# nvpro-samples/vk_gaussian_splatting

Measured on AMD Instinct MI355X. Metric: frames/s @1920x1080 + sorted Gsplats/s, garden-sized scene, higher is better.
Workload: dtype f32; 1 GPU; syn_garden N=5830000 x 1 instance(s) SH deg 3, storage sh/rgba format 0/0, 1920x1080, 64-pose orbit r=4 h=1.5 fov60, GPU radix sort, cull at dist (configs[2]); partition=single GPU

## Files before the change

vk_gaussian_splatting_amd/csrc/api_frame.hip:

```cpp
#include <cmath>

#include "scene_state.h"

int mgs_frame_set_occluder(MgsScene s, const float* depthDevice, const float* colorDevice, int width, int height)
{
  if(!s)
  {
    setError("mgs_frame_set_occluder: null handle");
    return MGS_ERR_INVALID_ARG;
  }
  if(!depthDevice)
  {
    s->occ.depth = s->occ.color = nullptr;
    s->occ.w = s->occ.h = 0;
    return MGS_OK;
  }
  if(width <= 0 || height <= 0)
  {
    setError("mgs_frame_set_occluder: width and height must be positive");
    return MGS_ERR_INVALID_ARG;
  }
  s->occ.depth = depthDevice;
  s->occ.color = colorDevice;
  s->occ.w     = width;
// ... 319 lines not shown
    if((rc = fb.pairVal0.ensure(cap))) return rc;
    if((rc = fb.pairKey1.ensure(cap))) return rc;
    if((rc = fb.chunkStart.ensure(cap / kPart + 4))) return rc;
    if((rc = fb.splatOffset.ensure(s->d->totalSplats))) return rc;
  }
  return ensureFrameImage(s, fp.p, F, std::max<uint32_t>(fp.nTiles, 256u), fp.occ.depth);
}

ProjectLaunch projectLaunch(MgsScene s, const FrameArgs& A, bool full, bool gpuSort)
{
  FrameBuffers& fb = s->fb;
  ProjectLaunch L{};
  L.dArgs           = fb.dArgs.p;
  L.totalPartitions = A.f.totalPartitions;
  L.full            = full;
  L.ctr             = fb.ctr.p;
  L.slotPairs       = fb.pairB.p;
  L.slotCount       = fb.slotCount.p;
  L.rec             = fb.rec.p;
  L.recGut          = fb.recGut.p;
  L.rect            = fb.rect.p;
  L.slotHist2       = fb.slotHist2.p;
  L.top16Rec        = fb.top16Rec.p;
  L.top16Count      = gpuSort ? fb.top16Count.p : nullptr;
  L.osPlan          = &fb.plans.p->os;
  L.order           = fb.prjOrder.p;
  return L;
}

static int issueSort(const FramePass& fp, hipStream_t st)
// ... 162 lines not shown
  return MGS_OK;
}

static GraphCache::Key graphKey(const FramePass& fp)
{
  const FrameConst& F = fp.A->f;
  GraphCache::Key   key;
  std::memset(&key, 0, sizeof(key));
  int32_t isoBits;
  std::memcpy(&isoBits, &F.depthIsoThreshold, 4);
  const int32_t kv[16] = {F.width, F.height, F.stripRow0, F.stripRow1, F.binShiftX, F.binShiftY, F.partitionCull, F.alphaMode,
                          F.debugFlags & (2 | 4), F.surfaceOutputs, fp.half, F.nInstances, F.shDegree, isoBits,
                          F.pipeline, F.stochastic | (F.dofMode << 1) | (F.temporalSampling << 2) | ((F.pipeline == 1 && F.kernelDegree != 2) ? 8 : 0) |
                              ((F.pipeline == 1 && F.normalMethod == 1) ? 16 : 0) |
                              (F.lightingMode << 5) |
                              (F.rideShift << 8) | (F.rideShapes << 16) | (F.rideSplit << 24)};
  std::memcpy(key.v, kv, sizeof(kv));
  key.p[0] = fp.s->fb.image.p;
  key.p[1] = fp.s->surf.depth.p;
  key.p[2] = fp.occ.depth;
  key.p[3] = fp.occ.color;
  return key;
}

static int launchFrame(const FramePass& fp, bool timed)
{
  GraphCache& graphs = fp.s->graphs;
  if(tuning().useGraph && graphs.ok && !timed && !fp.cpuMode)
  {
    const GraphCache::Key key  = graphKey(fp);
    hipGraphExec_t        exec = graphs.find(key);
// ... 367 lines not shown
```

vk_gaussian_splatting_amd/csrc/api_frameargs.hip:

```cpp
#include <cmath>

#include "scene_state.h"

void mgs_frame_params_default(MgsFrameParams* p)
{
  if(!p)
    return;
  std::memset(p, 0, sizeof(*p));
  const float id[16] = {1, 0, 0, 0, 0, 1, 0, 0, 0, 0, 1, 0, 0, 0, 0, 1};
  std::memcpy(p->view, id, sizeof(id));
  std::memcpy(p->proj, id, sizeof(id));
  p->width                = 1920;
  p->height               = 1080;
  p->splat_scale          = 1.0f;
  p->frustum_dilation     = 0.2f;
  p->alpha_cull_threshold = 1.0f / 255.0f;
  p->sh_degree            = 3;
  p->sort_mode            = MGS_SORT_GPU_RADIX;
  p->frustum_culling      = MGS_CULL_AT_DIST;
  p->target_format        = MGS_TARGET_RGBA16F;
  p->alpha_mode           = MGS_ALPHA_COVERAGE;
  p->size_culling_min_pixels = 1.0f;
  p->cpu_lazy_sort           = 1;
  p->thin_particle_threshold = 1e-6f;
// ... 126 lines not shown
  F.binsX     = (F.tilesX + (1 << bsx) - 1) >> bsx;
  F.binsY     = (F.tilesY + (1 << bsy) - 1) >> bsy;
  return MGS_OK;
}

static void fillInstanceConst(const MgsFrameParams* p, const Instance& I, const DeviceSet& d, InstanceConst& C)
{
  C.centers = d.centers;
  C.cov6    = d.cov6;
  C.rgba    = d.rgba;
  C.sh      = d.sh;
  C.partBox = d.partBox;
  C.maxScale = d.maxScale;
  C.scales    = d.scales;
  C.alpha     = d.alpha;
  C.rgbaF32   = d.rgbaF32;
  C.rotations = d.rotations;
  {
    auto len3 = [&](int c) { return std::sqrt((I.M[4 * c] * I.M[4 * c] + I.M[4 * c + 1] * I.M[4 * c + 1]) + I.M[4 * c + 2] * I.M[4 * c + 2]); };
    C.modelAxisMax = std::max(len3(0), std::max(len3(1), len3(2)));
  }
  std::memcpy(C.model, I.M, sizeof(C.model));
  mat4Mul(p->view, I.M, C.modelView);
  float inv[16], cam[4] = {p->camera_pos[0], p->camera_pos[1], p->camera_pos[2], 1.0f}, cm[4];
  mat4Inverse(I.M, inv);
  std::memcpy(C.modelInv, inv, sizeof(inv));
  mat4MulVec4(inv, cam, cm);
  C.camModel[0]  = cm[0];
  C.camModel[1]  = cm[1];
  C.camModel[2]  = cm[2];
// ... 139 lines not shown
  F.totalPartitions = s->d->totalParts;
  F.partitionCull   = F.cullMode == MGS_CULL_AT_DIST ? 1 : 0;
  uint32_t offset = 0, block = 0;
  for(int k = 0; k < F.nInstances; ++k)
  {
    const DeviceSet& d = s->d->sets[s->d->instances[k].set];
    InstanceConst&   C = A.inst[k];
    fillInstanceConst(p, s->d->instances[k], d, C);
    C.globalOffset = offset;
    C.blockBegin   = block;
    C.shDegree     = d.shDegree;
    C.shStride     = d.shPitch;
    offset += d.count;
    block += (d.count + kPart - 1) / kPart;
  }
  return MGS_OK;
}
```

vk_gaussian_splatting_amd/csrc/api_scene.hip:

```cpp
#include <cmath>

#include "scene_state.h"

static void materialDefault(MgsMaterial& m)
{
  std::memset(&m, 0, sizeof(m));
  m.emission[0] = m.emission[1] = m.emission[2] = 1.0f;
}
static MaterialDev materialToDevice(const MgsMaterial& m)
{
  MaterialDev d{};
  std::memcpy(d.ambient, m.ambient, 12);
  std::memcpy(d.diffuse, m.diffuse, 12);
  std::memcpy(d.specular, m.specular, 12);
  std::memcpy(d.emission, m.emission, 12);
  d.shininess = m.shininess;
  auto len = [](const float* v) { return std::sqrt(v[0] * v[0] + v[1] * v[1] + v[2] * v[2]); };
  d.needShading = (len(m.diffuse) > 0.001f || len(m.ambient) > 0.001f || len(m.specular) > 0.001f) ? 1 : 0;
  return d;
}

static int mgs_scene_create_impl(int device, MgsScene* out)
{
  if(!out)
  {
    setError("mgs_scene_create: null argument");
    return MGS_ERR_INVALID_ARG;
  }
  int count = 0;
  if(hipGetDeviceCount(&count) != hipSuccess || count == 0)
  {
    setError("mgs_scene_create: no HIP device available — the MI355X path has no CPU fallback");
    return MGS_ERR_DEVICE;
  }
  if(device < 0 || device >= count)
  {
// ... 41 lines not shown
}
int mgs_scene_create(int device, MgsScene* out)
{
  return guarded("mgs_scene_create", [&] { return mgs_scene_create_impl(device, out); });
}

static void freeSet(DeviceSet& d)
{
  if(d.centers) (void)hipFree(d.centers);
  if(d.cov6) (void)hipFree(d.cov6);
  if(d.rgba) (void)hipFree(d.rgba);
  if(d.sh) (void)hipFree(d.sh);
  if(d.partBox) (void)hipFree(d.partBox);
  if(d.maxScale) (void)hipFree(d.maxScale);
  if(d.alpha) (void)hipFree(d.alpha);
  if(d.rgbaF32 && (void*)d.rgbaF32 != d.rgba) (void)hipFree(d.rgbaF32);
  d.rgbaF32 = nullptr;
  if(d.scales) (void)hipFree(d.scales);
  if(d.rotations) (void)hipFree(d.rotations);
  d.centers = d.cov6 = d.partBox = d.maxScale = d.scales = d.rotations = d.alpha = nullptr;
  d.rgba = d.sh = nullptr;
  d.shFormat = d.rgbaFormat = -1;
}

SceneData::~SceneData()
{
  (void)hipSetDevice(device);
  for(auto& d : sets)
    freeSet(d);
  compInst.release();
  lightTab.release();
  for(auto& m : meshes)
    m.release();
  meshTab.release();
  bvh.release();
// ... 75 lines not shown
  {
    setError("mgs_scene_set_list_capacity: null scene");
    return MGS_ERR_INVALID_ARG;
  }
  s->listCapacityOverride = entries;
  s->wsEpoch              = ~0ull;
  return MGS_OK;
}

static uint64_t setBytes(const DeviceSet& d)
{
  if(!d.centers)
    return 0;
  const uint64_t n   = d.count;
  const uint64_t fmt[3] = {4, 2, 1};
  uint64_t       b   = n * (12 + 24 + 4 + 4 + 12 + 16) + ((n + kPart - 1) / kPart) * 32;
  b += n * 4 * fmt[d.rgbaFormat] + (d.rgbaFormat != MGS_FORMAT_FLOAT32 ? n * 16 : 0);
  b += d.sh ? n * (uint64_t)d.shPitch * fmt[d.shFormat] : 0;
  return b;
}
int mgs_scene_memory_usage(MgsScene s, uint64_t* sceneBytes, uint64_t* workingBytes)
{
  if(!s)
  {
    setError("mgs_scene_memory_usage: null scene");
    return MGS_ERR_INVALID_ARG;
  }
  if(sceneBytes)
  {
    uint64_t b = s->d->compInst.bytes() + s->d->lightTab.bytes() + s->d->meshTab.bytes() + s->d->bvh.bytes();
    for(const auto& m : s->d->meshes)
// ... 369 lines not shown
      std::vector<float> al(n);
      if(rgbaFormat != MGS_FORMAT_FLOAT32)
        parallelBatches(n * 4, [&](size_t i) {
          re[i] = rgbaFormat == MGS_FORMAT_FLOAT16 ? halfToFloat(floatToHalf(re[i])) : (float)toUint8(re[i], 0.f, 1.f) / 255.0f;
        });
      parallelBatches(n, [&](size_t i) { al[i] = re[4 * i + 3]; });
      if(rgbaFormat == MGS_FORMAT_FLOAT32)
        d.rgbaF32 = static_cast<float*>(d.rgba);
      else
      {
        HIPCHK(hipMalloc((void**)&d.rgbaF32, n * 4 * sizeof(float)));
        HIPCHK(hipMemcpy(d.rgbaF32, re.data(), n * 4 * sizeof(float), hipMemcpyHostToDevice));
      }
      HIPCHK(hipMalloc((void**)&d.alpha, n * sizeof(float)));
      HIPCHK(hipMemcpy(d.alpha, al.data(), n * sizeof(float), hipMemcpyHostToDevice));
    }
    if(d.shStride)
    {
      std::vector<float> sh, padded;
      buildShInterleaved(h, sh);
      d.shPitch = 48;
      padded.assign(n * (size_t)d.shPitch, 0.f);
      const int stride = d.shStride;
      parallelBatches(n, [&](size_t i) {
        std::memcpy(&padded[i * (size_t)d.shPitch], &sh[(size_t)perm[i] * (size_t)stride], sizeof(float) * stride);
      });
      int rc = uploadFormatted(padded, shFormat, true, &d.sh);
      if(rc != MGS_OK)
        return rc;
    }
// ... 255 lines not shown
```

vk_gaussian_splatting_amd/csrc/device_types.h:

```cpp
#pragma once
#include <cstdint>

namespace mgs {

constexpr int kMaxInstances       = 256;
constexpr int kMaxInlineInstances = 16;
constexpr int kMaxLights          = 64;
constexpr int kTilePx             = 16;

enum : uint32_t {
  kErrPairOverflow  = 1u << 0,
  kErrSpinTimeout   = 1u << 1,
  kErrSortOverflow  = 1u << 2,
};

struct InstanceConst
{
  const float* centers;
  const float* cov6;
  const void*  rgba;
  const float* rgbaF32;
  const float* alpha;
  const float* maxScale;
  const float* partBox;
  const void*  sh;
  const float* scales;
  const float* rotations;
  float        model[16];
  float        modelInv[16];
  float        modelView[16];
  float        camModel[3];
  float        modelAxisMax;
  float        modelScale;
  uint32_t     count;
  uint32_t     modelIsIdentity;
  uint32_t     modelIsAffine;
  uint32_t     globalOffset;
// ... 39 lines not shown
  float    gutFocal[2];
  float    gutMaxAngle;
  float    viewInv[16], projInv[16];
  int32_t  stochastic;
  int32_t  dofMode;
  int32_t  frameSampleId;
  int32_t  temporalSampling;
  float    focusDist, aperture;
  int32_t  kernelDegree;
  int32_t  normalMethod;
  int32_t  rideShift;
  int32_t  rideShapes;
  uint32_t rideEscape;
  int32_t  perspAffine;
  int32_t  rideSplit;
  int32_t  lightingMode;
  float    cameraPos[3];
  float    lightViewInv[16], lightProjInv[16];
};

struct FrameArgs
{
  FrameConst    f;
  InstanceConst inst[kMaxInstances];
};

struct CompositeArgs
{
  int32_t width, height;
  int32_t tilesX;
// ... 222 lines not shown
```

vk_gaussian_splatting_amd/csrc/k_project.hip:

```cpp
#include <cstdio>
#include <cstdlib>
#include <vector>
#include "kernels_common.h"
#include "launchers.h"
#include "slot_emit.h"
#include "partition_cull.h"

namespace mgs {

#ifndef MGS_PRJ_THREADS
#define MGS_PRJ_THREADS 256
#endif
constexpr int kPrjThreads = MGS_PRJ_THREADS;
constexpr int kPrjWaves   = kPrjThreads / 64;
constexpr int kPrjItems   = 2048 / kPrjThreads;
constexpr int kPrjPart    = kPrjThreads * kPrjItems;
static_assert(kPrjItems * kPrjWaves == 32 && kPrjPart == 2048, "the round x wave table of scanRoundWaveCounts has 32 entries");

struct Projected
{
  SplatRec rec;
  uint32_t rect;
};

struct SplatFetch
{
  float  alpha;
  float  px, py, pz;
  float4 cA;
  float2 cB;
};
__device__ __forceinline__ SplatFetch fetchSplat(const InstanceConst& I, uint32_t li)
{
  SplatFetch f;
  f.alpha = I.alpha[li];
  f.px  = I.centers[3 * (size_t)li + 0];
  f.py  = I.centers[3 * (size_t)li + 1];
  f.pz  = I.centers[3 * (size_t)li + 2];
  f.cA  = reinterpret_cast<const float4*>(I.cov6)[li];
  f.cB  = reinterpret_cast<const float2*>(I.cov6 + 4 * (size_t)I.count)[li];
  return f;
}

__device__ __forceinline__ float fastRcp(float x) { return __builtin_amdgcn_rcpf(x); }
__device__ __forceinline__ float fastSqrt(float x) { return __builtin_amdgcn_sqrtf(x); }

__device__ __forceinline__ bool projectSplat(const FrameConst& F, const InstanceConst& I, int instIdx, const SplatFetch& in,
                                             Projected& out)
{
  float4       col = make_float4(0.f, 0.f, 0.f, in.alpha);
  const float  px = in.px, py = in.py, pz = in.pz;
  const float4 cA = in.cA;
  const float2 cB = in.cB;

  bool         ok = !(col.w < F.alphaCull);
  const float* MV = I.modelView;
  const float  tx = MV[0] * px + MV[4] * py + MV[8] * pz + MV[12];
  const float  ty = MV[1] * px + MV[5] * py + MV[9] * pz + MV[13];
  const float  tz = MV[2] * px + MV[6] * py + MV[10] * pz + MV[14];
  const float* P  = F.proj;
  float        tw, cx, cy, cz, cw;
  if(F.perspAffine && (I.modelIsIdentity | I.modelIsAffine))
  {
    tw = 1.0f;
    cx = P[0] * tx + P[8] * tz;
    cy = P[5] * ty + P[9] * tz;
    cz = P[10] * tz + P[14];
    cw = P[11] * tz;
  }
  else
  {
    tw = MV[3] * px + MV[7] * py + MV[11] * pz + MV[15];
    cx = P[0] * tx + P[4] * ty + P[8] * tz + P[12] * tw;
    cy = P[1] * tx + P[5] * ty + P[9] * tz + P[13] * tw;
    cz = P[2] * tx + P[6] * ty + P[10] * tz + P[14] * tw;
    cw = P[3] * tx + P[7] * ty + P[11] * tz + P[15] * tw;
  }
  if(F.cullMode == 2)
  {
    const float c = (1.0f + F.frustumDilation) * cw;
    ok            = ok && !(fabsf(cx) > c || fabsf(cy) > c || cz < (0.0f - F.frustumDilation) * cw || cz > cw);
  }
  const float rw   = fastRcp(cw);
  const float ndcx = cx * rw, ndcy = cy * rw, ndcz = cz * rw;
  ok = ok && (ndcz >= 0.0f && ndcz <= 1.0f);

  const float s00 = cA.x, s01 = cA.y, s02 = cA.z, s11 = cA.w, s12 = cB.x, s22 = cB.y;
  const float rz = fastRcp(tz), rz2 = rz * rz;
  const float j00 = F.focal[0] * rz, j02 = -(F.focal[0] * tx) * rz2;
  const float j11 = F.focal[1] * rz, j12 = -(F.focal[1] * ty) * rz2;
  const float t00 = j00 * MV[0] + j02 * MV[2], t01 = j00 * MV[4] + j02 * MV[6], t02 = j00 * MV[8] + j02 * MV[10];
  const float t10 = j11 * MV[1] + j12 * MV[2], t11 = j11 * MV[5] + j12 * MV[6], t12 = j11 * MV[9] + j12 * MV[10];
  const float u0 = t00 * s00 + t01 * s01 + t02 * s02, u1 = t00 * s01 + t01 * s11 + t02 * s12,
              u2 = t00 * s02 + t01 * s12 + t02 * s22;
  const float v0 = t10 * s00 + t11 * s01 + t12 * s02, v1 = t10 * s01 + t11 * s11 + t12 * s12,
              v2 = t10 * s02 + t11 * s12 + t12 * s22;
  float a = u0 * t00 + u1 * t01 + u2 * t02;
  float b = u0 * t10 + u1 * t11 + u2 * t12;
  float d = v0 * t10 + v1 * t11 + v2 * t12;

  float detOrig = 0.f;
  if(F.msAA)
    detOrig = a * d - b * b;
  a += 0.3f;
  d += 0.3f;
  if(F.msAA)
  {
    const float detBlur = a * d - b * b;
    col.w *= fastSqrt(fmaxf(detOrig * fastRcp(detBlur), 0.0f));
  }
  const float D     = a * d - b * b;
  const float half  = 0.5f * (a + d);
  const float term2 = fastSqrt(fmaxf(0.1f, half * half - D));
  float ev1 = half + term2, ev2 = half - term2;
  ok        = ok && !(ev2 <= 0.0f);
  if(F.debugFlags & 1)
    ev1 = ev2 = 0.2f;
  float       e1x = (fabsf(b) < 0.001f) ? 1.0f : b, e1y = ev1 - a;
  const float el  = __builtin_amdgcn_rsqf(e1x * e1x + e1y * e1y);
  e1x *= el;
  e1y *= el;
  const float kSqrt8 = 2.8284271247461903f;
  const float l1     = F.splatScale * fminf(kSqrt8 * fastSqrt(ev1), 2048.0f);
  const float l2     = F.splatScale * fminf(kSqrt8 * fastSqrt(fmaxf(ev2, 0.f)), 2048.0f);
  ok                 = ok && (l1 > 0.f && l2 > 0.f);
  const float b1x = e1x * l1, b1y = e1y * l1;
  const float b2x = e1y * l2, b2y = -e1x * l2;

  const bool  noGauss = (F.debugFlags & 4) != 0;
  const float a255    = col.w * 255.0f;
  ok                  = ok && (noGauss || a255 > 1.0f);
  const float qmax    = noGauss ? 4.0f : fminf(4.0f, __builtin_amdgcn_logf(fmaxf(a255, 1.0f)) * 0.6931471805599453f + 1e-3f);
  const float shrink = fastSqrt(qmax * 0.25f) * 1.0005f;
  const float ex = shrink * fastSqrt(b1x * b1x + b2x * b2x) + 0.01f;
  const float ey = shrink * fastSqrt(b1y * b1y + b2y * b2y) + 0.01f;

  const float pcx = (ndcx + 1.0f) * 0.5f * (float)F.width;
  const float pcy = (ndcy + 1.0f) * 0.5f * (float)F.height;
  const float fx0 = ceilf(pcx - ex - 0.5f), fx1 = floorf(pcx + ex - 0.5f);
  const float fy0 = ceilf(pcy - ey - 0.5f), fy1 = floorf(pcy + ey - 0.5f);
  const float ymin = (float)(F.stripRow0 * kTilePx), ymax = (float)(min(F.stripRow1 * kTilePx, F.height) - 1);
  ok = ok && (fx1 >= fx0 && fy1 >= fy0 && fx1 >= 0.f && fx0 <= (float)(F.width - 1) && fy1 >= ymin && fy0 <= ymax);
  if(!ok)
    return false;
  const int x0 = (int)fmaxf(fx0, 0.f), x1 = (int)fminf(fx1, (float)(F.width - 1));
  const int y0 = (int)fmaxf(fy0, ymin), y1 = (int)fminf(fy1, ymax);
  const int sx = 4 + F.binShiftX, sy = 4 + F.binShiftY;
  out.rect = (uint32_t)(x0 >> sx) | ((uint32_t)(y0 >> sy) << 8) | ((uint32_t)(x1 >> sx) << 16) | ((uint32_t)(y1 >> sy) << 24);

  const float n1 = 2.0f * fastRcp(b1x * b1x + b1y * b1y), n2 = 2.0f * fastRcp(b2x * b2x + b2y * b2y);
  out.rec.cx  = pcx;
  out.rec.cy  = pcy;
  out.rec.p1x = b1x * n1;
  out.rec.p1y = b1y * n1;
  out.rec.p2x = b2x * n2;
  out.rec.p2y = b2y * n2;
  out.rec.a   = col.w;
  {
    const __half2 h = __halves2half2(__float2half_ru(ex), __float2half_ru(ey));
    out.rec.exey    = *reinterpret_cast<const uint32_t*>(&h);
  }
  return true;
}

#ifdef MGS_PRJ_TRACE
__device__ uint64_t* g_prjTrace = nullptr;
#define MGS_PRJ_STAMP(i) if(threadIdx.x == 0) trc[i] = wall_clock64();
#else
#define MGS_PRJ_STAMP(i)
#endif
template <bool FULL>
__global__ __launch_bounds__(kPrjThreads, 6) void k_project(const FrameArgs* __restrict__ Ap, FrameCounters* __restrict__ ctr,
                                                         uint2* __restrict__ slotPairs, uint32_t* __restrict__ slotCount,
                                                         SplatRec* __restrict__ rec, uint32_t* __restrict__ rect,
                                                         uint32_t* __restrict__ slotHist2,
                                                         uint32_t* __restrict__ top16Rec, uint32_t* __restrict__ top16Count,
                                                         OsPlan* __restrict__ osPlan, const uint32_t* __restrict__ order)
{
  const FrameArgs& A = *Ap;
#ifdef MGS_PRJ_TRACE
  __shared__ uint64_t trc[8];
  if(threadIdx.x < 8) trc[threadIdx.x] = 0;
  MGS_PRJ_STAMP(0)
#endif
  __shared__ __attribute__((aligned(16))) unsigned char s_raw[12288 + 4096 + 8192];
  float4(*s_rec)[64 * 3] = reinterpret_cast<float4(*)[64 * 3]>(s_raw);
  uint16_t* s_li         = reinterpret_cast<uint16_t*>(s_raw + 12288);
  uint32_t* s_key        = reinterpret_cast<uint32_t*>(s_raw + 16384);
  __shared__ uint32_t s_small[256];
  __shared__ uint32_t s_cnt[32];
  __shared__ uint32_t s_base[33];
  EmitLds E;
  E.li    = s_li;
  E.key   = s_key;
// ... 3 lines not shown
  E.start = reinterpret_cast<uint16_t*>(s_small + 128);
  E.stage = reinterpret_cast<uint2*>(s_raw);
  E.cnt   = s_cnt;

  const int      t = threadIdx.x, lane = laneId(), w = t >> 6;
  const uint32_t part = order[blockIdx.x];
  int            k    = 0;
  for(int i = 1; i < A.f.nInstances; ++i)
    if(part >= A.inst[i].blockBegin)
      k = i;
  const InstanceConst& I      = A.inst[k];
  const uint32_t       local0 = (part - I.blockBegin) * kPrjPart;

  const PartitionBox pbox = partitionLoad(I, part - I.blockBegin);
  float px[kPrjItems], py[kPrjItems], pz[kPrjItems];
  const bool stripMode = FULL && A.f.partitionCull && (A.f.stripRow1 - A.f.stripRow0) < A.f.tilesY;
  [[maybe_unused]] float msc[kPrjItems];
#pragma unroll
  for(int it = 0; it < kPrjItems; ++it)
  {
    const uint32_t li = min(local0 + it * kPrjThreads + t, I.count - 1u);
    px[it] = I.centers[3 * (size_t)li];
    py[it] = I.centers[3 * (size_t)li + 1];
    pz[it] = I.centers[3 * (size_t)li + 2];
    if constexpr(FULL)
    {
      msc[it] = 0.0f;
      if(stripMode)
        msc[it] = I.maxScale[li];
    }
  }
  float          partRadius = 3.0e38f;
  const uint32_t pflag      = A.f.partitionCull ? partitionTest(A, I, pbox, partRadius) : 0u;
  if(pflag & 1u)
  {
    emitEmptySlot<kPrjThreads>(slotCount, slotHist2, top16Rec, part);
    return;
  }
  uint32_t key[kPrjItems];
  uint64_t bal[kPrjItems];
  bool     vis[kPrjItems];
#ifdef MGS_PRJ_TRACE
  if(px[0] + py[1] + pz[2] == 12345.678f) trc[7] = 1;
  MGS_PRJ_STAMP(1)
#endif
  const bool identityFast = (pflag & 4u) != 0u && I.modelIsIdentity != 0u;
  const bool w1Fast = (pflag & 12u) == 12u && A.f.perspAffine != 0 && (I.modelIsIdentity != 0u || I.modelIsAffine != 0u);
  const bool  stripPre = stripMode;
  const float stripR   = stripPre ? partRadius : 3.0e38f;
  const float stripK   = fmaxf(fabsf(A.f.focal[0]), fabsf(A.f.focal[1])) * I.modelScale * 2.8284271247461903f;
  const bool  gutFish  = A.f.cameraModel == 1 && A.f.pipeline == 1;
  const float stripY0  = (float)(A.f.stripRow0 * kTilePx), stripY1 = (float)min(A.f.stripRow1 * kTilePx, A.f.height);
  const bool  insideFast = (pflag & 2u) != 0u && A.f.cullMode == 1 && !stripPre;
#pragma unroll
  for(int it = 0; it < kPrjItems; ++it)
  {
    const uint32_t li = local0 + it * kPrjThreads + t;
    float          wp[4], vp[4], cp[4];
    if(identityFast)
    {
#pragma clang fp contract(off)
      wp[0] = px[it] + 0.0f;
      wp[1] = py[it] + 0.0f;
      wp[2] = pz[it] + 0.0f;
      wp[3] = 1.0f;
    }
    else if(w1Fast)
    {
// ... 16 lines not shown
      if(w1Fast)
        mulPerspExactW1ZW(A.f.proj, vp[2], cp[2], cp[3]);
      else
        mulMat4ExactZW(A.f.proj, vp[0], vp[1], vp[2], vp[3], cp[2], cp[3]);
      nz = divExact(cp[2], cp[3]);
    }
    else
    {
      if(w1Fast)
      {
        mulPerspExactW1XY(A.f.proj, vp[0], vp[1], vp[2], cp[0], cp[1]);
        mulPerspExactW1ZW(A.f.proj, vp[2], cp[2], cp[3]);
      }
      else
        mulMat4Exact(A.f.proj, vp[0], vp[1], vp[2], vp[3], cp);
      const float nx = divExact(cp[0], cp[3]), ny = divExact(cp[1], cp[3]);
      nz             = divExact(cp[2], cp[3]);
      if(A.f.cullMode == 1 && distStageCulled(A.f, nx, ny, nz, vp[0], vp[1], vp[2]))
        v = false;
      if(stripPre)
      {
        float R = stripR;
        if constexpr(FULL)
        {
          const float zv = -vp[2];
          if(zv > 1.0e-4f && !gutFish)
          {
            const float iz = fastRcp(zv), qx = vp[0] * iz, qy = vp[1] * iz;
            const float kk = fastSqrt(2.0f + qx * qx + qy * qy);
            float       Ri = A.f.splatScale * (kk * stripK * msc[it] * iz + 3.2f);
            Ri             = fminf(Ri, 2897.0f * A.f.splatScale) * 1.01f + 2.0f;
            R              = fminf(R, Ri);
          }
        }
        const float ypx = (ny + 1.0f) * 0.5f * (float)A.f.height;
        if(ypx + R < stripY0 || ypx - R > stripY1)
          v = false;
      }
    }
    if(A.f.sizeCulling && v)
      v = !sizeCulled(I.maxScale[min(li, I.count - 1u)], A.f.splatScale, I.modelAxisMax, vp[2], A.f.maxFocal,
                      A.f.sizeCullingMinPixels);
    vis[it] = v;
    key[it] = A.f.frontToBack ? encodeKey(nz) : encodeKey(-nz);
    bal[it] = __ballot(v);
    if(lane == 0)
      s_cnt[it * kPrjWaves + w] = (uint32_t)__popcll(bal[it]);
  }
  MGS_PRJ_STAMP(2)
  const uint32_t M = scanRoundWaveCounts(s_cnt, s_base);
#pragma unroll
  for(int it = 0; it < kPrjItems; ++it)
    if(vis[it])
    {
      const uint32_t pos = s_base[it * kPrjWaves + w] + lanesBelow(bal[it]);
// ... 11 lines not shown
    return;
  }
  if constexpr(!FULL)
  {
    E.code = nullptr;
    emitSlot<kPrjThreads, kPrjItems>(M, true, E, slotPairs, slotCount, slotHist2, top16Rec, top16Count, osPlan, ctr, part, I.globalOffset + local0);
    return;
  }
  else
  {
    SplatFetch cur;
    uint32_t   liCur = 0;
    if(t < M)
    {
      liCur = local0 + s_li[t];
      cur   = fetchSplat(I, liCur);
    }
    static_assert(kPrjItems == 8, "RideCodes holds eight rounds");
    RideCodes      codes;
    bool           anySurvivor = false;
    const uint32_t rideShift = (uint32_t)A.f.rideShift;
    for(uint32_t j0 = 0; j0 < M; j0 += kPrjThreads)
    {
      uint32_t       code = 0u;
      const uint32_t j    = j0 + t;
      uint32_t       gidOk = 0xFFFFFFFFu;
      SplatFetch     nxt;
      uint32_t       liNxt = 0;
      const bool     haveNxt = j + kPrjThreads < M;
      liNxt = local0 + s_li[haveNxt ? j + kPrjThreads : 0u];
      liNxt = min(liNxt, I.count - 1u);
      nxt   = fetchSplat(I, liNxt);
      if(j < M)
      {
        const uint32_t li = liCur;
        Projected      pr;
        if(projectSplat(A.f, I, k, cur, pr))
        {
          gidOk       = I.globalOffset + li;
          float4* dst = &s_rec[w][lane * 3];
          dst[0]      = make_float4(pr.rec.cx, pr.rec.cy, pr.rec.p1x, pr.rec.p1y);
          dst[1]      = make_float4(pr.rec.p2x, pr.rec.p2y, pr.rec.a, __uint_as_float(pr.rec.exey));
          if(rideShift != 0u)
            code = rideEncode(pr.rect, A.f.binsX, A.f.binsY, A.f.rideShapes, A.f.rideEscape);
          if(rideShift == 0u || code == A.f.rideEscape)
            rect[gidOk] = pr.rect;
          s_li[j] |= 0x8000u;
          anySurvivor = true;
        }
      }
      reinterpret_cast<uint32_t*>(&s_rec[w][lane * 3 + 2])[0] = gidOk;
      __builtin_amdgcn_wave_barrier();
#pragma unroll
      for(int i = 0; i < 2; ++i)
      {
        const int      rr = 32 * i + (lane >> 1), part = lane & 1;
        const uint32_t g  = reinterpret_cast<const uint32_t*>(&s_rec[w][rr * 3 + 2])[0];
        if(g != 0xFFFFFFFFu)
          reinterpret_cast<float4*>(rec + g)[part] = s_rec[w][rr * 3 + part];
      }
// ... 9 lines not shown
    if(!anyOut)
    {
      emitEmptySlot<kPrjThreads>(slotCount, slotHist2, top16Rec, part);
#ifdef MGS_PRJ_TRACE
      MGS_PRJ_STAMP(5)
      if(threadIdx.x == 0 && g_prjTrace)
      {
        uint64_t* o = g_prjTrace + (size_t)blockIdx.x * 8;
        for(int i = 0; i < 6; ++i) o[i] = trc[i];
        o[6] = M;
        o[7] = 0;
      }
#endif
      return;
    }
    if(rideShift != 0u)
    {
      uint16_t* s_code = reinterpret_cast<uint16_t*>(s_raw);
#pragma unroll
      for(int r = 0; r < kPrjItems; ++r)
        s_code[r * kPrjThreads + t] = (uint16_t)codes.get(r);
    }
    const uint32_t outCount = emitSlot<kPrjThreads, kPrjItems>(M, false, E, slotPairs, slotCount, slotHist2, top16Rec, top16Count, osPlan, ctr, part,
                                                               I.globalOffset + local0, rideShift | (A.f.rideSplit ? 0x100u : 0u));
    (void)outCount;
#ifdef MGS_PRJ_TRACE
    MGS_PRJ_STAMP(5)
    if(threadIdx.x == 0 && g_prjTrace)
    {
      uint64_t* o = g_prjTrace + (size_t)blockIdx.x * 8;
      for(int i = 0; i < 6; ++i) o[i] = trc[i];
// ... 14 lines not shown
  const bool full = L.full;
#ifdef MGS_PRJ_TRACE
  static uint64_t* traceBuf = nullptr;
  const char*      tracePath = std::getenv("MGS_PRJ_TRACE_FILE");
  const size_t     traceN = (size_t)L.totalPartitions * 8;
  if(tracePath && full)
  {
    if(!traceBuf)
    {
      (void)hipMalloc(&traceBuf, (size_t)1 << 24);
      (void)hipMemcpyToSymbol(HIP_SYMBOL(g_prjTrace), &traceBuf, sizeof(traceBuf));
    }
    (void)hipMemsetAsync(traceBuf, 0, traceN * 8, stream);
  }
#endif
#define MGS_LAUNCH(FULLV)                                                                                                \
  hipLaunchKernelGGL((k_project<FULLV>), grid, block, 0, stream, L.dArgs, L.ctr, L.slotPairs, L.slotCount, L.rec, L.rect, \
                     L.slotHist2, L.top16Rec, L.top16Count, L.osPlan, L.order)
  if(full)
    MGS_LAUNCH(true);
  else
    MGS_LAUNCH(false);
#undef MGS_LAUNCH
#ifdef MGS_PRJ_TRACE
  if(tracePath && full)
  {
    (void)hipStreamSynchronize(stream);
    std::vector<uint64_t> h(traceN);
    (void)hipMemcpy(h.data(), traceBuf, traceN * 8, hipMemcpyDeviceToHost);
    if(FILE* fp = std::fopen(tracePath, "wb"))
    {
      std::fwrite(h.data(), 8, traceN, fp);
      std::fclose(fp);
    }
  }
#endif
}
// ... 3 lines not shown
```

vk_gaussian_splatting_amd/csrc/kernels_common.h:

```cpp
#pragma once
#include <hip/hip_runtime.h>
#include <hip/hip_fp16.h>

#include <cstdint>

#include "device_types.h"

namespace mgs {

constexpr int kWave = 64;

__device__ __forceinline__ int laneId() { return (int)__lane_id(); }

__device__ __forceinline__ uint32_t lanesBelow(uint64_t mask)
{
  return __builtin_amdgcn_mbcnt_hi((uint32_t)(mask >> 32), __builtin_amdgcn_mbcnt_lo((uint32_t)mask, 0u));
}

__device__ __forceinline__ uint32_t waveSum(uint32_t v)
{
#pragma unroll
  for(int o = 32; o > 0; o >>= 1)
    v += __shfl_xor(v, o, 64);
  return v;
// ... 247 lines not shown
  return (theta < F.gutMaxAngle) && (ox > -tx) && (oy > -ty) && (ox < resx + tx) && (oy < resy + ty);
}

__device__ __forceinline__ bool distStageCulled(const FrameConst& F, float nx, float ny, float nz, float vx, float vy, float vz)
{
  if(F.cameraModel == 1)
  {
    if(!fisheyeCullValid(F, vx, vy, vz))
      return true;
    return nz < 0.f - F.frustumDilation || nz > 1.0f;
  }
  const float c = 1.0f + F.frustumDilation;
  return fabsf(nx) > c || fabsf(ny) > c || nz < 0.f - F.frustumDilation || nz > 1.0f;
}

__device__ __host__ __forceinline__ uint32_t rngXxhash32(uint32_t px, uint32_t py, uint32_t pz)
{
  const uint32_t p0 = 2246822519u, p1 = 3266489917u, p2 = 668265263u, p3 = 374761393u;
  uint32_t       h  = pz + p3 + px * p1;
  h                 = p2 * ((h << 17) | (h >> 15));
  h += py * p1;
  h = p2 * ((h << 17) | (h >> 15));
  h = p0 * (h ^ (h >> 15));
  h = p1 * (h ^ (h >> 13));
  return h ^ (h >> 16);
}
__device__ __host__ __forceinline__ uint32_t rngPcg(uint32_t& state)
{
  const uint32_t prev = state * 747796405u + 2891336453u;
  const uint32_t word = ((prev >> ((prev >> 28u) + 4u)) ^ prev) * 277803737u;
// ... 11 lines not shown
```

vk_gaussian_splatting_amd/csrc/launchers.h:

```cpp
#pragma once
#include <hip/hip_runtime.h>

#include <cstdint>

#include "compare_types.h"
#include "device_types.h"
#include "frame_state.h"
#include "sort_plan.h"

namespace mgs {

constexpr uint32_t kPart = 2048;

struct ProjectLaunch
{
  const FrameArgs* dArgs;
  uint32_t         totalPartitions;
  bool             full;
  FrameCounters*   ctr;
  uint2*           slotPairs;
  uint32_t*        slotCount;
  SplatRec*        rec;
  GutRec*          recGut;
  uint32_t*        rect;
  uint32_t*        slotHist2;
  uint32_t*        top16Rec;
  uint32_t*        top16Count;
  OsPlan*          osPlan;
  const uint32_t*  order;
};
void launchProject(hipStream_t stream, const ProjectLaunch& L);
void launchProjectGut(hipStream_t stream, const ProjectLaunch& L);

// ... 80 lines not shown
```

vk_gaussian_splatting_amd/csrc/scene_state.h:

```cpp
#pragma once
#include <hip/hip_runtime.h>
#include <rccl/rccl.h>

#include <algorithm>
#include <condition_variable>
#include <cstddef>
#include <cstring>
#include <map>
#include <memory>
#include <mutex>
#include <stdexcept>
#include <string>
#include <thread>
#include <vector>

#include "../../include/mgs.h"
#include "host_model.h"
#include "launchers.h"
#include "tuning.h"

using namespace mgs;

#define HIPCHK(expr)                                                                                                    \
  do                                                                                                                    \
// ... 41 lines not shown
};

struct DeviceSet
{
  std::shared_ptr<HostSplatSet> host;
  float*   centers = nullptr;
  float*   cov6    = nullptr;
  void*    rgba    = nullptr;
  void*    sh      = nullptr;
  uint32_t count   = 0;
  int      shDegree = 0, shStride = 0;
  int      shPitch = 0;
  int      shFormat = -1, rgbaFormat = -1;
  float*   maxScale = nullptr;
  float*   rgbaF32 = nullptr;
  float*   alpha = nullptr;
  float*   scales = nullptr;
  float*   rotations = nullptr;
  float*   partBox = nullptr;
  std::vector<uint32_t> newToOld, oldToNew;
};

struct Instance
{
  int   set;
  float M[16];
};

template <typename T>
struct DevBuf
// ... 496 lines not shown
```

vk_gaussian_splatting_amd/csrc/tuning.h:

```cpp
#pragma once
#include <cstdint>
#include <optional>
#include <string>

namespace mgs {

struct Tuning
{
  bool directBin       = true;
  bool rectRide        = true;
  bool rideSplitAlways = false;
  int  dbTranspose     = 1;
  bool binAdapt        = true;
  bool binShiftSet     = false;
  std::optional<int> binShiftX, binShiftY;
  std::optional<uint64_t> pairCapacity;
  bool exactShortcuts  = true;
  bool     sortRemap       = true;
  bool     rawSortGeneric  = false;
  uint32_t osFlat          = 1;
  uint32_t osPartMin       = 1536;
  uint32_t meshWorkItems = 1u << 20;
  bool useGraph = true;
  std::optional<std::string> rcclLib;
};

const Tuning& tuning();

}
```

vk_gaussian_splatting_amd/csrc/tuning.hip:

```cpp
#include "tuning.h"

#include <cstdio>
#include <cstdlib>
#include <cstring>

#include "sort_plan.h"

namespace mgs {

static Tuning readTuning()
{
  Tuning t;
  auto flag = [](const char* name, bool dflt) {
    const char* e = std::getenv(name);
    return e ? std::atoi(e) != 0 : dflt;
  };
  t.directBin      = flag("MGS_DIRECT_BIN", true);
  t.rectRide       = flag("MGS_RECT_RIDE", true);
  t.exactShortcuts = flag("MGS_EXACT_SHORTCUTS", true);
  t.sortRemap      = flag("MGS_SORT_REMAP", true);
  t.useGraph       = flag("MGS_GRAPH", true);
  if(const char* e = std::getenv("MGS_RIDE_SPLIT"))
    t.rideSplitAlways = std::atoi(e) == 2;
  if(const char* e = std::getenv("MGS_DB_TRANSPOSE"))
    t.dbTranspose = std::atoi(e);
  if(const char* e = std::getenv("MGS_BIN_SHIFT"))
  {
    int       x = 0, y = 0;
    const int got = std::sscanf(e, "%d,%d", &x, &y);
    t.binShiftSet = true;
    if(got >= 1)
      t.binShiftX = x;
    if(got >= 2)
      t.binShiftY = y;
// ... 33 lines not shown
```

Baseline: 3827 frames/s.

## Add specialized projection kernel variants, opacity shrink table, and banded XY cull

Adds template specializations of the projection kernel: a 'plain' mode that compiles out generic branches (strip mode, size culling, debug flags, non-affine perspective) and a table mode that reads a per-splat precomputed opacity shrink factor instead of computing log/sqrt every frame. It also adds a banded frustum cull that uses a fast reciprocal to classify points clearly inside or outside and skips the exact divisions when a whole wavefront is certain. The plain mode is off by default, so only the banded cull runs by default; the table costs one extra float per splat of memory and a load-time kernel.

```diff
diff --git a/vk_gaussian_splatting_amd/csrc/api_frame.hip b/vk_gaussian_splatting_amd/csrc/api_frame.hip
--- a/vk_gaussian_splatting_amd/csrc/api_frame.hip
+++ b/vk_gaussian_splatting_amd/csrc/api_frame.hip
@@ -357,6 +357,7 @@
   L.dArgs           = fb.dArgs.p;
   L.totalPartitions = A.f.totalPartitions;
   L.full            = full;
+  L.mode            = A.f.projMode;
   L.ctr             = fb.ctr.p;
   L.slotPairs       = fb.pairB.p;
   L.slotCount       = fb.slotCount.p;
@@ -549,7 +550,7 @@
                           F.pipeline, F.stochastic | (F.dofMode << 1) | (F.temporalSampling << 2) | ((F.pipeline == 1 && F.kernelDegree != 2) ? 8 : 0) |
                               ((F.pipeline == 1 && F.normalMethod == 1) ? 16 : 0) |
                               (F.lightingMode << 5) |
-                              (F.rideShift << 8) | (F.rideShapes << 16) | (F.rideSplit << 24)};
+                              (F.rideShift << 8) | (F.rideShapes << 16) | (F.rideSplit << 24) | (F.projMode << 25)};
   std::memcpy(key.v, kv, sizeof(kv));
   key.p[0] = fp.s->fb.image.p;
   key.p[1] = fp.s->surf.depth.p;
diff --git a/vk_gaussian_splatting_amd/csrc/api_frameargs.hip b/vk_gaussian_splatting_amd/csrc/api_frameargs.hip
--- a/vk_gaussian_splatting_amd/csrc/api_frameargs.hip
+++ b/vk_gaussian_splatting_amd/csrc/api_frameargs.hip
@@ -164,6 +164,7 @@
   C.maxScale = d.maxScale;
   C.scales    = d.scales;
   C.alpha     = d.alpha;
+  C.shrink    = d.shrink;
   C.rgbaF32   = d.rgbaF32;
   C.rotations = d.rotations;
   {
@@ -333,5 +334,18 @@
     offset += d.count;
     block += (d.count + kPart - 1) / kPart;
   }
+  {
+    bool plain = tuning().prjPlain && F.perspAffine != 0 && F.msAA == 0 && (F.debugFlags & 5) == 0 && F.cullMode == MGS_CULL_AT_DIST
+                 && F.sizeCulling == 0 && F.stripRow0 == 0 && F.stripRow1 == F.tilesY && F.pipeline == MGS_PIPELINE_3DGS
+                 && F.cameraModel == MGS_CAMERA_PINHOLE && F.rideShift != 0;
+    bool table = tuning().prjOpacityTable;
+    for(int k = 0; k < F.nInstances; ++k)
+    {
+      plain = plain && (A.inst[k].modelIsIdentity | A.inst[k].modelIsAffine) != 0u;
+      table = table && A.inst[k].shrink != nullptr;
+    }
+    F.projMode   = plain ? (table ? 3 : 1) : 0;
+    F.bandedCull = tuning().prjBandedCull ? 1 : 0;
+  }
   return MGS_OK;
 }
diff --git a/vk_gaussian_splatting_amd/csrc/api_scene.hip b/vk_gaussian_splatting_amd/csrc/api_scene.hip
--- a/vk_gaussian_splatting_amd/csrc/api_scene.hip
+++ b/vk_gaussian_splatting_amd/csrc/api_scene.hip
@@ -1,5 +1,6 @@
 #include <cmath>
 
+#include "kernels_common.h"
 #include "scene_state.h"
 
 static void materialDefault(MgsMaterial& m)
@@ -20,6 +21,13 @@
   return d;
 }
 
+__global__ void k_opacity_shrink_table(const float* __restrict__ alpha, float* __restrict__ shrink, uint32_t n)
+{
+  const uint32_t i = blockIdx.x * 256u + threadIdx.x;
+  if(i < n)
+    shrink[i] = mgs::opacityShrinkEntry(alpha[i]);
+}
+
 static int mgs_scene_create_impl(int device, MgsScene* out)
 {
   if(!out)
@@ -91,11 +99,12 @@
   if(d.partBox) (void)hipFree(d.partBox);
   if(d.maxScale) (void)hipFree(d.maxScale);
   if(d.alpha) (void)hipFree(d.alpha);
+  if(d.shrink) (void)hipFree(d.shrink);
   if(d.rgbaF32 && (void*)d.rgbaF32 != d.rgba) (void)hipFree(d.rgbaF32);
   d.rgbaF32 = nullptr;
   if(d.scales) (void)hipFree(d.scales);
   if(d.rotations) (void)hipFree(d.rotations);
-  d.centers = d.cov6 = d.partBox = d.maxScale = d.scales = d.rotations = d.alpha = nullptr;
+  d.centers = d.cov6 = d.partBox = d.maxScale = d.scales = d.rotations = d.alpha = d.shrink = nullptr;
   d.rgba = d.sh = nullptr;
   d.shFormat = d.rgbaFormat = -1;
 }
@@ -201,7 +210,7 @@
     return 0;
   const uint64_t n   = d.count;
   const uint64_t fmt[3] = {4, 2, 1};
-  uint64_t       b   = n * (12 + 24 + 4 + 4 + 12 + 16) + ((n + kPart - 1) / kPart) * 32;
+  uint64_t       b   = n * (12 + 24 + 4 + 4 + 4 + 12 + 16) + ((n + kPart - 1) / kPart) * 32;
   b += n * 4 * fmt[d.rgbaFormat] + (d.rgbaFormat != MGS_FORMAT_FLOAT32 ? n * 16 : 0);
   b += d.sh ? n * (uint64_t)d.shPitch * fmt[d.shFormat] : 0;
   return b;
@@ -601,6 +610,13 @@
       }
       HIPCHK(hipMalloc((void**)&d.alpha, n * sizeof(float)));
       HIPCHK(hipMemcpy(d.alpha, al.data(), n * sizeof(float), hipMemcpyHostToDevice));
+      HIPCHK(hipMalloc((void**)&d.shrink, n * sizeof(float)));
+      if(n)
+      {
+        hipLaunchKernelGGL(k_opacity_shrink_table, dim3((unsigned)((n + 255) / 256)), dim3(256), 0, nullptr, d.alpha, d.shrink, (uint32_t)n);
+        HIPCHK(hipGetLastError());
+        HIPCHK(hipStreamSynchronize(nullptr));
+      }
     }
     if(d.shStride)
     {
diff --git a/vk_gaussian_splatting_amd/csrc/device_types.h b/vk_gaussian_splatting_amd/csrc/device_types.h
--- a/vk_gaussian_splatting_amd/csrc/device_types.h
+++ b/vk_gaussian_splatting_amd/csrc/device_types.h
@@ -21,6 +21,7 @@
   const void*  rgba;
   const float* rgbaF32;
   const float* alpha;
+  const float* shrink;
   const float* maxScale;
   const float* partBox;
   const void*  sh;
@@ -90,6 +91,8 @@
   uint32_t rideEscape;
   int32_t  perspAffine;
   int32_t  rideSplit;
+  int32_t  projMode;
+  int32_t  bandedCull;
   int32_t  lightingMode;
   float    cameraPos[3];
   float    lightViewInv[16], lightProjInv[16];
diff --git a/vk_gaussian_splatting_amd/csrc/k_project.hip b/vk_gaussian_splatting_amd/csrc/k_project.hip
--- a/vk_gaussian_splatting_amd/csrc/k_project.hip
+++ b/vk_gaussian_splatting_amd/csrc/k_project.hip
@@ -26,14 +26,20 @@
 struct SplatFetch
 {
   float  alpha;
+  float  shrink;
   float  px, py, pz;
   float4 cA;
   float2 cB;
 };
+constexpr int kPrjPlain = 1, kPrjTable = 2;
+template <int MODE>
 __device__ __forceinline__ SplatFetch fetchSplat(const InstanceConst& I, uint32_t li)
 {
   SplatFetch f;
   f.alpha = I.alpha[li];
+  f.shrink = 0.0f;
+  if constexpr((MODE & kPrjTable) != 0)
+    f.shrink = I.shrink[li];
   f.px  = I.centers[3 * (size_t)li + 0];
   f.py  = I.centers[3 * (size_t)li + 1];
   f.pz  = I.centers[3 * (size_t)li + 2];
@@ -45,9 +51,12 @@
 __device__ __forceinline__ float fastRcp(float x) { return __builtin_amdgcn_rcpf(x); }
 __device__ __forceinline__ float fastSqrt(float x) { return __builtin_amdgcn_sqrtf(x); }
 
+template <int MODE>
 __device__ __forceinline__ bool projectSplat(const FrameConst& F, const InstanceConst& I, int instIdx, const SplatFetch& in,
                                              Projected& out)
 {
+  constexpr bool PLAIN = (MODE & kPrjPlain) != 0, TABLE = (MODE & kPrjTable) != 0;
+  static_assert(PLAIN || !TABLE, "the opacity table stands for the plain frame's opacity chain only (msAA rescales alpha per frame)");
   float4       col = make_float4(0.f, 0.f, 0.f, in.alpha);
   const float  px = in.px, py = in.py, pz = in.pz;
   const float4 cA = in.cA;
@@ -60,7 +69,7 @@
   const float  tz = MV[2] * px + MV[6] * py + MV[10] * pz + MV[14];
   const float* P  = F.proj;
   float        tw, cx, cy, cz, cw;
-  if(F.perspAffine && (I.modelIsIdentity | I.modelIsAffine))
+  if(PLAIN || (F.perspAffine && (I.modelIsIdentity | I.modelIsAffine)))
   {
     tw = 1.0f;
     cx = P[0] * tx + P[8] * tz;
@@ -76,7 +85,7 @@
     cz = P[2] * tx + P[6] * ty + P[10] * tz + P[14] * tw;
     cw = P[3] * tx + P[7] * ty + P[11] * tz + P[15] * tw;
   }
-  if(F.cullMode == 2)
+  if(!PLAIN && F.cullMode == 2)
   {
     const float c = (1.0f + F.frustumDilation) * cw;
     ok            = ok && !(fabsf(cx) > c || fabsf(cy) > c || cz < (0.0f - F.frustumDilation) * cw || cz > cw);
@@ -99,12 +108,13 @@
   float b = u0 * t10 + u1 * t11 + u2 * t12;
   float d = v0 * t10 + v1 * t11 + v2 * t12;
 
+  const bool msAA = F.msAA != 0;
   float detOrig = 0.f;
-  if(F.msAA)
+  if(msAA)
     detOrig = a * d - b * b;
   a += 0.3f;
   d += 0.3f;
-  if(F.msAA)
+  if(msAA)
   {
     const float detBlur = a * d - b * b;
     col.w *= fastSqrt(fmaxf(detOrig * fastRcp(detBlur), 0.0f));
@@ -114,7 +124,7 @@
   const float term2 = fastSqrt(fmaxf(0.1f, half * half - D));
   float ev1 = half + term2, ev2 = half - term2;
   ok        = ok && !(ev2 <= 0.0f);
-  if(F.debugFlags & 1)
+  if(!PLAIN && (F.debugFlags & 1))
     ev1 = ev2 = 0.2f;
   float       e1x = (fabsf(b) < 0.001f) ? 1.0f : b, e1y = ev1 - a;
   const float el  = __builtin_amdgcn_rsqf(e1x * e1x + e1y * e1y);
@@ -127,11 +137,20 @@
   const float b1x = e1x * l1, b1y = e1y * l1;
   const float b2x = e1y * l2, b2y = -e1x * l2;
 
-  const bool  noGauss = (F.debugFlags & 4) != 0;
-  const float a255    = col.w * 255.0f;
-  ok                  = ok && (noGauss || a255 > 1.0f);
-  const float qmax    = noGauss ? 4.0f : fminf(4.0f, __builtin_amdgcn_logf(fmaxf(a255, 1.0f)) * 0.6931471805599453f + 1e-3f);
-  const float shrink = fastSqrt(qmax * 0.25f) * 1.0005f;
+  float shrink;
+  if constexpr(TABLE)
+  {
+    shrink = in.shrink;
+    ok     = ok && shrink >= 0.0f;
+  }
+  else
+  {
+    const bool  noGauss = !PLAIN && (F.debugFlags & 4) != 0;
+    const float a255    = col.w * 255.0f;
+    ok                  = ok && (noGauss || a255 > 1.0f);
+    const float qmax    = noGauss ? 4.0f : opacityQmax(a255);
+    shrink              = opacityShrink(qmax);
+  }
   const float ex = shrink * fastSqrt(b1x * b1x + b2x * b2x) + 0.01f;
   const float ey = shrink * fastSqrt(b1y * b1y + b2y * b2y) + 0.01f;
 
@@ -139,7 +158,7 @@
   const float pcy = (ndcy + 1.0f) * 0.5f * (float)F.height;
   const float fx0 = ceilf(pcx - ex - 0.5f), fx1 = floorf(pcx + ex - 0.5f);
   const float fy0 = ceilf(pcy - ey - 0.5f), fy1 = floorf(pcy + ey - 0.5f);
-  const float ymin = (float)(F.stripRow0 * kTilePx), ymax = (float)(min(F.stripRow1 * kTilePx, F.height) - 1);
+  const float ymin = PLAIN ? 0.0f : (float)(F.stripRow0 * kTilePx), ymax = PLAIN ? (float)(F.height - 1) : (float)(min(F.stripRow1 * kTilePx, F.height) - 1);
   ok = ok && (fx1 >= fx0 && fy1 >= fy0 && fx1 >= 0.f && fx0 <= (float)(F.width - 1) && fy1 >= ymin && fy0 <= ymax);
   if(!ok)
     return false;
@@ -169,7 +188,7 @@
 #else
 #define MGS_PRJ_STAMP(i)
 #endif
-template <bool FULL>
+template <bool FULL, int MODE>
 __global__ __launch_bounds__(kPrjThreads, 6) void k_project(const FrameArgs* __restrict__ Ap, FrameCounters* __restrict__ ctr,
                                                          uint2* __restrict__ slotPairs, uint32_t* __restrict__ slotCount,
                                                          SplatRec* __restrict__ rec, uint32_t* __restrict__ rect,
@@ -178,6 +197,9 @@
                                                          OsPlan* __restrict__ osPlan, const uint32_t* __restrict__ order)
 {
   const FrameArgs& A = *Ap;
+  constexpr bool   PLAIN = (MODE & kPrjPlain) != 0;
+  constexpr bool   BAND  = PLAIN || !FULL;
+  static_assert(FULL || MODE == 0, "the keys-only kernel has the generic instantiation only");
 #ifdef MGS_PRJ_TRACE
   __shared__ uint64_t trc[8];
   if(threadIdx.x < 8) trc[threadIdx.x] = 0;
@@ -211,7 +233,7 @@
 
   const PartitionBox pbox = partitionLoad(I, part - I.blockBegin);
   float px[kPrjItems], py[kPrjItems], pz[kPrjItems];
-  const bool stripMode = FULL && A.f.partitionCull && (A.f.stripRow1 - A.f.stripRow0) < A.f.tilesY;
+  const bool stripMode = FULL && !PLAIN && A.f.partitionCull && (A.f.stripRow1 - A.f.stripRow0) < A.f.tilesY;
   [[maybe_unused]] float msc[kPrjItems];
 #pragma unroll
   for(int it = 0; it < kPrjItems; ++it)
@@ -228,7 +250,7 @@
     }
   }
   float          partRadius = 3.0e38f;
-  const uint32_t pflag      = A.f.partitionCull ? partitionTest(A, I, pbox, partRadius) : 0u;
+  const uint32_t pflag      = (PLAIN || A.f.partitionCull) ? partitionTest(A, I, pbox, partRadius) : 0u;
   if(pflag & 1u)
   {
     emitEmptySlot<kPrjThreads>(slotCount, slotHist2, top16Rec, part);
@@ -242,13 +264,17 @@
   MGS_PRJ_STAMP(1)
 #endif
   const bool identityFast = (pflag & 4u) != 0u && I.modelIsIdentity != 0u;
-  const bool w1Fast = (pflag & 12u) == 12u && A.f.perspAffine != 0 && (I.modelIsIdentity != 0u || I.modelIsAffine != 0u);
+  const bool w1Fast = (pflag & 12u) == 12u && (PLAIN || (A.f.perspAffine != 0 && (I.modelIsIdentity != 0u || I.modelIsAffine != 0u)));
   const bool  stripPre = stripMode;
   const float stripR   = stripPre ? partRadius : 3.0e38f;
   const float stripK   = fmaxf(fabsf(A.f.focal[0]), fabsf(A.f.focal[1])) * I.modelScale * 2.8284271247461903f;
   const bool  gutFish  = A.f.cameraModel == 1 && A.f.pipeline == 1;
   const float stripY0  = (float)(A.f.stripRow0 * kTilePx), stripY1 = (float)min(A.f.stripRow1 * kTilePx, A.f.height);
-  const bool  insideFast = (pflag & 2u) != 0u && A.f.cullMode == 1 && !stripPre;
+  const bool  cullAtDist = PLAIN || A.f.cullMode == 1;
+  const bool  insideFast = (pflag & 2u) != 0u && cullAtDist && !stripPre;
+  const float cullC  = 1.0f + A.f.frustumDilation;
+  const bool  banded = BAND && A.f.bandedCull != 0 && cullAtDist && !stripPre && A.f.cameraModel != 1 && cullC >= kBandCMin && cullC <= kBandCMax;
+  const float bandHi = cullC * kBandHi, bandLo = cullC * kBandLo;
 #pragma unroll
   for(int it = 0; it < kPrjItems; ++it)
   {
@@ -295,31 +321,44 @@
       }
       else
         mulMat4Exact(A.f.proj, vp[0], vp[1], vp[2], vp[3], cp);
-      const float nx = divExact(cp[0], cp[3]), ny = divExact(cp[1], cp[3]);
-      nz             = divExact(cp[2], cp[3]);
-      if(A.f.cullMode == 1 && distStageCulled(A.f, nx, ny, nz, vp[0], vp[1], vp[2]))
-        v = false;
-      if(stripPre)
+      bool xyOut  = false;
+      bool unsure = true;
+      if(banded)
+        unsure = !bandedXYCull(cp[0], cp[1], cp[3], bandHi, bandLo, xyOut);
+      if(banded && __ballot(unsure) == 0ull)
       {
-        float R = stripR;
-        if constexpr(FULL)
-        {
-          const float zv = -vp[2];
-          if(zv > 1.0e-4f && !gutFish)
-          {
-            const float iz = fastRcp(zv), qx = vp[0] * iz, qy = vp[1] * iz;
-            const float kk = fastSqrt(2.0f + qx * qx + qy * qy);
-            float       Ri = A.f.splatScale * (kk * stripK * msc[it] * iz + 3.2f);
-            Ri             = fminf(Ri, 2897.0f * A.f.splatScale) * 1.01f + 2.0f;
-            R              = fminf(R, Ri);
-          }
-        }
-        const float ypx = (ny + 1.0f) * 0.5f * (float)A.f.height;
-        if(ypx + R < stripY0 || ypx - R > stripY1)
+        nz = divExact(cp[2], cp[3]);
+        if(xyOut || nz < 0.f - A.f.frustumDilation || nz > 1.0f)
           v = false;
       }
-    }
-    if(A.f.sizeCulling && v)
+      else
+      {
+        const float nx = divExact(cp[0], cp[3]), ny = divExact(cp[1], cp[3]);
+        nz             = divExact(cp[2], cp[3]);
+        if(cullAtDist && distStageCulled(A.f, nx, ny, nz, vp[0], vp[1], vp[2]))
+          v = false;
+        if(stripPre)
+        {
+          float R = stripR;
+          if constexpr(FULL)
+          {
+            const float zv = -vp[2];
+            if(zv > 1.0e-4f && !gutFish)
+            {
+              const float iz = fastRcp(zv), qx = vp[0] * iz, qy = vp[1] * iz;
+              const float kk = fastSqrt(2.0f + qx * qx + qy * qy);
+              float       Ri = A.f.splatScale * (kk * stripK * msc[it] * iz + 3.2f);
+              Ri             = fminf(Ri, 2897.0f * A.f.splatScale) * 1.01f + 2.0f;
+              R              = fminf(R, Ri);
+            }
+          }
+          const float ypx = (ny + 1.0f) * 0.5f * (float)A.f.height;
+          if(ypx + R < stripY0 || ypx - R > stripY1)
+            v = false;
+        }
+      }
+    }
+    if(!PLAIN && A.f.sizeCulling && v)
       v = !sizeCulled(I.maxScale[min(li, I.count - 1u)], A.f.splatScale, I.modelAxisMax, vp[2], A.f.maxFocal,
                       A.f.sizeCullingMinPixels);
     vis[it] = v;
@@ -361,12 +400,13 @@
     if(t < M)
     {
       liCur = local0 + s_li[t];
-      cur   = fetchSplat(I, liCur);
+      cur   = fetchSplat<MODE>(I, liCur);
     }
     static_assert(kPrjItems == 8, "RideCodes holds eight rounds");
     RideCodes      codes;
     bool           anySurvivor = false;
     const uint32_t rideShift = (uint32_t)A.f.rideShift;
+    const bool     ride      = PLAIN || rideShift != 0u;
     for(uint32_t j0 = 0; j0 < M; j0 += kPrjThreads)
     {
       uint32_t       code = 0u;
@@ -377,20 +417,20 @@
       const bool     haveNxt = j + kPrjThreads < M;
       liNxt = local0 + s_li[haveNxt ? j + kPrjThreads : 0u];
       liNxt = min(liNxt, I.count - 1u);
-      nxt   = fetchSplat(I, liNxt);
+      nxt   = fetchSplat<MODE>(I, liNxt);
       if(j < M)
       {
         const uint32_t li = liCur;
         Projected      pr;
-        if(projectSplat(A.f, I, k, cur, pr))
+        if(projectSplat<MODE>(A.f, I, k, cur, pr))
         {
           gidOk       = I.globalOffset + li;
           float4* dst = &s_rec[w][lane * 3];
           dst[0]      = make_float4(pr.rec.cx, pr.rec.cy, pr.rec.p1x, pr.rec.p1y);
           dst[1]      = make_float4(pr.rec.p2x, pr.rec.p2y, pr.rec.a, __uint_as_float(pr.rec.exey));
-          if(rideShift != 0u)
+          if(ride)
             code = rideEncode(pr.rect, A.f.binsX, A.f.binsY, A.f.rideShapes, A.f.rideEscape);
-          if(rideShift == 0u || code == A.f.rideEscape)
+          if(!ride || code == A.f.rideEscape)
             rect[gidOk] = pr.rect;
           s_li[j] |= 0x8000u;
           anySurvivor = true;
@@ -430,7 +470,7 @@
 #endif
       return;
     }
-    if(rideShift != 0u)
+    if(ride)
     {
       uint16_t* s_code = reinterpret_cast<uint16_t*>(s_raw);
 #pragma unroll
@@ -475,13 +515,17 @@
     (void)hipMemsetAsync(traceBuf, 0, traceN * 8, stream);
   }
 #endif
-#define MGS_LAUNCH(FULLV)                                                                                                \
-  hipLaunchKernelGGL((k_project<FULLV>), grid, block, 0, stream, L.dArgs, L.ctr, L.slotPairs, L.slotCount, L.rec, L.rect, \
+#define MGS_LAUNCH(FULLV, MODEV)                                                                                                \
+  hipLaunchKernelGGL((k_project<FULLV, MODEV>), grid, block, 0, stream, L.dArgs, L.ctr, L.slotPairs, L.slotCount, L.rec, L.rect, \
                      L.slotHist2, L.top16Rec, L.top16Count, L.osPlan, L.order)
-  if(full)
-    MGS_LAUNCH(true);
+  if(!full)
+    MGS_LAUNCH(false, 0);
+  else if(L.mode == (kPrjPlain | kPrjTable))
+    MGS_LAUNCH(true, kPrjPlain | kPrjTable);
+  else if(L.mode == kPrjPlain)
+    MGS_LAUNCH(true, kPrjPlain);
   else
-    MGS_LAUNCH(false);
+    MGS_LAUNCH(true, 0);
 #undef MGS_LAUNCH
 #ifdef MGS_PRJ_TRACE
   if(tracePath && full)
diff --git a/vk_gaussian_splatting_amd/csrc/kernels_common.h b/vk_gaussian_splatting_amd/csrc/kernels_common.h
--- a/vk_gaussian_splatting_amd/csrc/kernels_common.h
+++ b/vk_gaussian_splatting_amd/csrc/kernels_common.h
@@ -285,6 +285,29 @@
   return fabsf(nx) > c || fabsf(ny) > c || nz < 0.f - F.frustumDilation || nz > 1.0f;
 }
 
+constexpr float kBandHi = 1.00006103515625f, kBandLo = 0.99993896484375f;
+constexpr float kBandCMin = 8.6736173798840355e-19f, kBandCMax = 1.152921504606846976e18f;
+__device__ __forceinline__ bool bandedXYCull(float cx, float cy, float cw, float hi, float lo, bool& outside)
+{
+  const float aw  = fabsf(cw);
+  const bool  wOk = aw >= kBandCMin && aw <= kBandCMax;
+  const float r   = __builtin_amdgcn_rcpf(cw);
+  const float qx = fabsf(cx * r), qy = fabsf(cy * r);
+  outside        = qx > hi || qy > hi;
+  return wOk && (outside || (qx < lo && qy < lo));
+}
+
+__device__ __forceinline__ float opacityQmax(float a255)
+{
+  return fminf(4.0f, __builtin_amdgcn_logf(fmaxf(a255, 1.0f)) * 0.6931471805599453f + 1e-3f);
+}
+__device__ __forceinline__ float opacityShrink(float qmax) { return __builtin_amdgcn_sqrtf(qmax * 0.25f) * 1.0005f; }
+__device__ __forceinline__ float opacityShrinkEntry(float alpha)
+{
+  const float a255 = alpha * 255.0f;
+  return a255 > 1.0f ? opacityShrink(opacityQmax(a255)) : -1.0f;
+}
+
 __device__ __host__ __forceinline__ uint32_t rngXxhash32(uint32_t px, uint32_t py, uint32_t pz)
 {
   const uint32_t p0 = 2246822519u, p1 = 3266489917u, p2 = 668265263u, p3 = 374761393u;
diff --git a/vk_gaussian_splatting_amd/csrc/launchers.h b/vk_gaussian_splatting_amd/csrc/launchers.h
--- a/vk_gaussian_splatting_amd/csrc/launchers.h
+++ b/vk_gaussian_splatting_amd/csrc/launchers.h
@@ -17,6 +17,7 @@
   const FrameArgs* dArgs;
   uint32_t         totalPartitions;
   bool             full;
+  int              mode;
   FrameCounters*   ctr;
   uint2*           slotPairs;
   uint32_t*        slotCount;
diff --git a/vk_gaussian_splatting_amd/csrc/scene_state.h b/vk_gaussian_splatting_amd/csrc/scene_state.h
--- a/vk_gaussian_splatting_amd/csrc/scene_state.h
+++ b/vk_gaussian_splatting_amd/csrc/scene_state.h
@@ -79,6 +79,7 @@
   int      shFormat = -1, rgbaFormat = -1;
   float*   maxScale = nullptr;
   float*   rgbaF32 = nullptr;
+  float*   shrink = nullptr;
   float*   alpha = nullptr;
   float*   scales = nullptr;
   float*   rotations = nullptr;
diff --git a/vk_gaussian_splatting_amd/csrc/tuning.h b/vk_gaussian_splatting_amd/csrc/tuning.h
--- a/vk_gaussian_splatting_amd/csrc/tuning.h
+++ b/vk_gaussian_splatting_amd/csrc/tuning.h
@@ -16,6 +16,9 @@
   std::optional<int> binShiftX, binShiftY;
   std::optional<uint64_t> pairCapacity;
   bool exactShortcuts  = true;
+  bool prjPlain        = false;
+  bool prjOpacityTable = true;
+  bool prjBandedCull   = true;
   bool     sortRemap       = true;
   bool     rawSortGeneric  = false;
   uint32_t osFlat          = 1;
diff --git a/vk_gaussian_splatting_amd/csrc/tuning.hip b/vk_gaussian_splatting_amd/csrc/tuning.hip
--- a/vk_gaussian_splatting_amd/csrc/tuning.hip
+++ b/vk_gaussian_splatting_amd/csrc/tuning.hip
@@ -18,6 +18,9 @@
   t.directBin      = flag("MGS_DIRECT_BIN", true);
   t.rectRide       = flag("MGS_RECT_RIDE", true);
   t.exactShortcuts = flag("MGS_EXACT_SHORTCUTS", true);
+  t.prjPlain        = flag("MGS_PRJ_PLAIN", false);
+  t.prjOpacityTable = flag("MGS_PRJ_OPACITY_TABLE", true);
+  t.prjBandedCull   = flag("MGS_PRJ_BANDED_CULL", true);
   t.sortRemap      = flag("MGS_SORT_REMAP", true);
   t.useGraph       = flag("MGS_GRAPH", true);
   if(const char* e = std::getenv("MGS_RIDE_SPLIT"))
```

After: 3742 frames/s. 0.978x the previous value.
